# ALIZE-Speaker-Recognition/LIA_RAL

Measured on AMD Instinct MI355X. Metric: Gframe-Gaussian evals/s (UBM EM pass: LLK + full-posterior statistics), higher is better.
Workload: dtype f64; 1 GPU; TrainWorld EM: 2048-Gaussian diag UBM, 60-dim float32 frames, 10000000 frames per GPU resident in HBM, 1 EM iteration per step; gaussians=2048, dim=60, frames_per_gpu=10000000, partitioning=frames sharded per rank, one RCCL all-reduce of 247810 doubles per step

## Files before the change

lia_ral_amd/csrc/devutil.h:

```cpp
#pragma once
#include <hip/hip_runtime.h>
#include <stdint.h>

typedef double d4 __attribute__((ext_vector_type(4)));

#define MFMA_F64(a, b, c) __builtin_amdgcn_mfma_f64_16x16x4f64((a), (b), (c), 0, 0, 0)

#define GMMIV_NEG_BIG (-1.0e300)
#define GMMIV_ZERO_LLK (-745.1332191019412)
#define GMMIV_PAD_LOGIT (-1.0e9)

__device__ __forceinline__ double gexp(double x)
{
    x = fmax(x, -750.0);
    const double n = __builtin_rint(x * 1.4426950408889634074);
    double r = __builtin_fma(n, -6.93147180369123816490e-01, x);
    r = __builtin_fma(n, -1.90821492927058770002e-10, r);
    double p = 1.6059043836821613e-10;
    p = __builtin_fma(p, r, 2.08767569878681e-09);
    p = __builtin_fma(p, r, 2.505210838544172e-08);
    p = __builtin_fma(p, r, 2.755731922398589e-07);
    p = __builtin_fma(p, r, 2.7557319223985893e-06);
    p = __builtin_fma(p, r, 2.48015873015873e-05);
    p = __builtin_fma(p, r, 1.984126984126984e-04);
// ... 15 lines not shown
{
    x = fmax(x, -750.0);
    const double k = __builtin_rint(x * 46.16624130844683);
    double r = __builtin_fma(k, -0.021660849219188094, x);
    r = __builtin_fma(k, -1.733101967801894e-10, r);
    const int ki = (int)k;
    const double tj = tab[ki & 31];
    double p = 1.984126984126984e-04;
    p = __builtin_fma(p, r, 1.388888888888889e-03);
    p = __builtin_fma(p, r, 8.333333333333333e-03);
    p = __builtin_fma(p, r, 4.1666666666666664e-02);
    p = __builtin_fma(p, r, 1.6666666666666666e-01);
    p = __builtin_fma(p, r, 0.5);
    p = __builtin_fma(p, r, 1.0);
    p = p * r;
    return __builtin_ldexp(__builtin_fma(tj, p, tj), ki >> 5);
}

__device__ __forceinline__ double gexp_scaled(double x, int E, const double *tab)
{
    x = fmax(x, -4.0e7);
    const double k = __builtin_rint(x * 46.16624130844683);
    double r = __builtin_fma(k, -0.021660849219188094, x);
    r = __builtin_fma(k, -1.733101967801894e-10, r);
    const int ki = (int)k;
    const double tj = tab[ki & 31];
    double p = 1.984126984126984e-04;
    p = __builtin_fma(p, r, 1.388888888888889e-03);
    p = __builtin_fma(p, r, 8.333333333333333e-03);
    p = __builtin_fma(p, r, 4.1666666666666664e-02);
    p = __builtin_fma(p, r, 1.6666666666666666e-01);
    p = __builtin_fma(p, r, 0.5);
    p = __builtin_fma(p, r, 1.0);
    p = p * r;
    int n = (ki >> 5) - E;
    n = n < -2000 ? -2000 : n;
    return __builtin_ldexp(__builtin_fma(tj, p, tj), n);
}
#ifndef GEXP_TAB_BITS
#define GEXP_TAB_BITS 11
#endif
#define GEXP_TAB_N (1 << GEXP_TAB_BITS)
#if GEXP_TAB_BITS == 11
#define GEXP_TAB_SCALE 2954.639443740597
#define GEXP_TAB_HI 0.00033845076904981397
#define GEXP_TAB_LO 2.7079718246904592e-12
#define GEXP_TAB_LN2N 0.00033845077175778578
#elif GEXP_TAB_BITS == 6
#define GEXP_TAB_SCALE 92.33248261689366
#define GEXP_TAB_HI 0.010830424609594047
#define GEXP_TAB_LO 8.66550983900947e-11
#define GEXP_TAB_LN2N 0.010830424696249145
#else
#error "GEXP_TAB_BITS must be 6 or 11"
#endif
__device__ __forceinline__ void gexp_tab_init(double *tab, int tid, int nthreads)
{
    for (int j = tid; j < GEXP_TAB_N; j += nthreads) tab[j] = exp2((double)j * (1.0 / GEXP_TAB_N));
}
__device__ __forceinline__ double gexp_tab_poly(double r)
{
#if GEXP_TAB_BITS == 11
    double p = 1.6666666666666666e-01;
#else
    double p = 8.333333333333333e-03;
    p = __builtin_fma(p, r, 4.1666666666666664e-02);
    p = __builtin_fma(p, r, 1.6666666666666666e-01);
#endif
    p = __builtin_fma(p, r, 0.5);
    p = __builtin_fma(p, r, 1.0);
    return p * r;
}
__device__ __forceinline__ void gexp_tab_reduce(double x, int &ki, double &r)
{
    const double k = __builtin_rint(x * GEXP_TAB_SCALE);
#ifdef GEXP_TAB_TWO_STEP
    r = __builtin_fma(k, -GEXP_TAB_HI, x);
    r = __builtin_fma(k, -GEXP_TAB_LO, r);
#else
    r = __builtin_fma(k, -GEXP_TAB_LN2N, x);
#endif
    ki = (int)k;
}
__device__ __forceinline__ double gexp_tab_finish(int ki, double r, int E, const double *tab)
{
    const double tj = tab[ki & (GEXP_TAB_N - 1)];
    return __builtin_ldexp(__builtin_fma(tj, gexp_tab_poly(r), tj), (ki >> GEXP_TAB_BITS) - E);
}
__device__ __forceinline__ double gexp_tab_scaled(double x, int E, const double *tab)
{
    int ki;
    double r;
    gexp_tab_reduce(x, ki, r);
    return gexp_tab_finish(ki, r, E, tab);
}
__device__ __forceinline__ int gexp_tab_exponent(double x)
{
    return ((int)__builtin_rint(x * GEXP_TAB_SCALE)) >> GEXP_TAB_BITS;
}
__device__ __forceinline__ int gexp_exponent(double x)
{
    x = fmax(x, -4.0e7);
    return ((int)__builtin_rint(x * 46.16624130844683)) >> 5;
}

template <int CTRL> __device__ __forceinline__ int dpp_i32(int v) { return __builtin_amdgcn_update_dpp(0, v, CTRL, 0xf, 0xf, false); }
__device__ __forceinline__ int row_max_i32(int v)
{
    int o;
    o = dpp_i32<0x128>(v); v = o > v ? o : v;
    o = dpp_i32<0x124>(v); v = o > v ? o : v;
    o = dpp_i32<0x122>(v); v = o > v ? o : v;
    o = dpp_i32<0x121>(v); v = o > v ? o : v;
    return v;
}

__device__ __forceinline__ int row_min_i32(int v)
{
    int o;
    o = dpp_i32<0x128>(v); v = o < v ? o : v;
    o = dpp_i32<0x124>(v); v = o < v ? o : v;
    o = dpp_i32<0x122>(v); v = o < v ? o : v;
    o = dpp_i32<0x121>(v); v = o < v ? o : v;
    return v;
}

__device__ __forceinline__ void wave_argmax_f64(double &v, int &c)
{
#define GMMIV_ARGMAX_STEP(CTRL)                                                                    \
    {                                                                                              \
        const int ohi = dpp_i32<CTRL>(__double2hiint(v)), olo = dpp_i32<CTRL>(__double2loint(v)); \
        const int oc = dpp_i32<CTRL>(c);                                                           \
        const double ov = __hiloint2double(ohi, olo);                                              \
        if (ov > v || (ov == v && oc < c)) { v = ov; c = oc; }                                     \
    }
    GMMIV_ARGMAX_STEP(0x128)
    GMMIV_ARGMAX_STEP(0x124)
    GMMIV_ARGMAX_STEP(0x122)
    GMMIV_ARGMAX_STEP(0x121)
#undef GMMIV_ARGMAX_STEP
    const double v0 = __hiloint2double(__builtin_amdgcn_readlane(__double2hiint(v), 0), __builtin_amdgcn_readlane(__double2loint(v), 0));
    const int c0 = __builtin_amdgcn_readlane(c, 0);
    double wv = v0;
    int wc = c0;
#pragma unroll
    for (int r = 1; r < 4; ++r) {
        const double ov = __hiloint2double(__builtin_amdgcn_readlane(__double2hiint(v), 16 * r), __builtin_amdgcn_readlane(__double2loint(v), 16 * r));
        const int oc = __builtin_amdgcn_readlane(c, 16 * r);
        if (ov > wv || (ov == wv && oc < wc)) { wv = ov; wc = oc; }
    }
    v = wv;
    c = wc;
}

__device__ __forceinline__ double dpp_f64_0x128(double v) { return __hiloint2double(dpp_i32<0x128>(__double2hiint(v)), dpp_i32<0x128>(__double2loint(v))); }
__device__ __forceinline__ double dpp_f64_0x124(double v) { return __hiloint2double(dpp_i32<0x124>(__double2hiint(v)), dpp_i32<0x124>(__double2loint(v))); }
__device__ __forceinline__ double dpp_f64_0x122(double v) { return __hiloint2double(dpp_i32<0x122>(__double2hiint(v)), dpp_i32<0x122>(__double2loint(v))); }
__device__ __forceinline__ double dpp_f64_0x121(double v) { return __hiloint2double(dpp_i32<0x121>(__double2hiint(v)), dpp_i32<0x121>(__double2loint(v))); }
__device__ __forceinline__ double readlane_f64u(double v, int l)
{
    return __hiloint2double(__builtin_amdgcn_readlane(__double2hiint(v), l), __builtin_amdgcn_readlane(__double2loint(v), l));
}
__device__ __forceinline__ double wave_sum_f64_dpp(double v)
{
    v += dpp_f64_0x128(v); v += dpp_f64_0x124(v); v += dpp_f64_0x122(v); v += dpp_f64_0x121(v);
    return (readlane_f64u(v, 0) + readlane_f64u(v, 16)) + (readlane_f64u(v, 32) + readlane_f64u(v, 48));
}
__device__ __forceinline__ double half_sum_f64_dpp(double v, bool hi)
{
    v += dpp_f64_0x128(v); v += dpp_f64_0x124(v); v += dpp_f64_0x122(v); v += dpp_f64_0x121(v);
// ... 75 lines not shown
```

lia_ral_amd/csrc/gmm_kernels.hip:

```cpp
#include <atomic>
#include "devutil.h"
#include "lds_attr.h"
#include "gmm_kernels.h"

typedef double d2v __attribute__((ext_vector_type(2)));

__device__ __forceinline__ void gmm_const_one(int c, int C, int D, const double *__restrict__ w, const double *__restrict__ mean,
                                              const double *__restrict__ iv, double *__restrict__ a, double *__restrict__ logwcst)
{
    if (c >= C) { a[c] = GMMIV_NEG_BIG; logwcst[c] = GMMIV_NEG_BIG; return; }
    double sl = 0.0, sm = 0.0;
    for (int d = 0; d < D; ++d) {
        double v = iv[(size_t)c * D + d], m = mean[(size_t)c * D + d];
        sl += log(v);
        sm += m * m * v;
    }
    double lw = (w[c] > 0.0) ? log(w[c]) : GMMIV_NEG_BIG;
    double lc = lw - 0.5 * D * 1.8378770664093454836 + 0.5 * sl;
    lc = fmax(lc, GMMIV_NEG_BIG);
    logwcst[c] = lc;
    a[c] = fmax(lc - 0.5 * sm, GMMIV_NEG_BIG);
}
__global__ void k_gmm_const(int C, int Cp, int D, const double *__restrict__ w,
                            const double *__restrict__ mean, const double *__restrict__ iv,
                            double *__restrict__ a, double *__restrict__ logwcst)
{
    int c = blockIdx.x * blockDim.x + threadIdx.x;
    if (c >= Cp) return;
    gmm_const_one(c, C, D, w, mean, iv, a, logwcst);
}
__global__ void k_gmm_const_batch(int C, int Cp, int D, const double *__restrict__ w, long sw, const double *__restrict__ mean, long sm,
                                  const double *__restrict__ iv, long si, double *__restrict__ a, double *__restrict__ logwcst)
{
    const int c = blockIdx.x * blockDim.x + threadIdx.x;
    const size_t g = blockIdx.y;
    if (c >= Cp) return;
    gmm_const_one(c, C, D, w + g * sw, mean + g * sm, iv + g * si, a + g * Cp, logwcst + g * Cp);
}

__device__ __forceinline__ double gmm_pack_one(long e, int C, int D, int KS, const double *__restrict__ mean,
                                               const double *__restrict__ iv, const double *__restrict__ a)
{
    const int NR = 2 * KS + 2;
    int lane = e & 63;
    int row = (e >> 6) % NR;
    int ct = (e >> 6) / NR;
    int j = lane & 15, q = lane >> 4;
    int c = ct * 16 + j;
    double v = 0.0;
    if (row < 2 * KS) {
        int s = row < KS ? row : row - KS;
        int k = 4 * s + q;
        if (c < C && k < D) {
            double ivv = iv[(size_t)c * D + k];
            v = row < KS ? mean[(size_t)c * D + k] * ivv : -0.5 * ivv;
        }
    } else if (row == 2 * KS) {
        v = c < C ? fmax(a[c], GMMIV_PAD_LOGIT) : GMMIV_PAD_LOGIT;
    } else {
        v = q == 0 ? (c < C ? fmax(a[c], GMMIV_PAD_LOGIT) : GMMIV_PAD_LOGIT) : (q == 1 ? -1.0 : 0.0);
    }
    return v;
}
__global__ void k_gmm_pack(int C, int D, int KS, int nct, const double *__restrict__ mean,
                           const double *__restrict__ iv, const double *__restrict__ a,
                           double *__restrict__ Pt)
{
    long e = (long)blockIdx.x * blockDim.x + threadIdx.x;
    long total = (long)nct * (2 * KS + 2) * 64;
    if (e >= total) return;
    Pt[e] = gmm_pack_one(e, C, D, KS, mean, iv, a);
}
__global__ void k_gmm_pack_batch(int C, int Cp, int D, int KS, int nct, const int *__restrict__ ids, const double *__restrict__ mean, long sm,
                                 const double *__restrict__ iv, long si, const double *__restrict__ a, double *__restrict__ Pt)
{
    long e = (long)blockIdx.x * blockDim.x + threadIdx.x;
    long total = (long)nct * (2 * KS + 2) * 64;
    if (e >= total) return;
    const size_t g = (size_t)ids[blockIdx.y];
    Pt[(size_t)blockIdx.y * total + e] = gmm_pack_one(e, C, D, KS, mean + g * sm, iv + g * si, a + g * Cp);
}

__global__ void k_gmm_transpose(int C, int Cp, int D, const double *__restrict__ mean,
                                const double *__restrict__ iv, double *__restrict__ meanT,
                                double *__restrict__ ivT)
{
    long e = (long)blockIdx.x * blockDim.x + threadIdx.x;
    if (e >= (long)D * Cp) return;
    int c = e % Cp, d = e / Cp;
    meanT[e] = c < C ? mean[(size_t)c * D + d] : 0.0;
    ivT[e] = c < C ? iv[(size_t)c * D + d] : 0.0;
}

#define TOPC_CAP 256
#define GMMIV_MIN_FRAME_EXP (-1076)
#ifndef K1_ABL
#define K1_ABL 0
#endif
#ifndef K1_PLAIN_SHARED
#define K1_PLAIN_SHARED 1
#endif
template <int KS, typename XT, int NW, int MODE, bool MM = false>
__global__ __launch_bounds__(NW * 64, 2) void k_llk_mfma(const void *__restrict__ x, long T, long ldx, int D,
                                                  const double *__restrict__ Pt, int nct,
                                                  double *__restrict__ lse_out, int use_glds, int dbg,
                                                  double *__restrict__ zbuf, long nfb, int *__restrict__ eit,
                                                  double *__restrict__ inv_out, int *__restrict__ efin_out,
                                                  const gmmiv_model_tile *__restrict__ tiles, long pt_stride)
{
    constexpr bool WZ = MODE == 1, TC = MODE == 2;
    static_assert(!MM || (MODE != 2 && NW == 8), "a model per segment: plain and stored-likelihood modes, 8 waves");
    constexpr int NR = 2 * KS + 2;
    constexpr int GT = 2;
    constexpr int TILE_D = GT * NR * 64;
    constexpr int PIECES = TILE_D * 8 / 1024;
    extern __shared__ __attribute__((aligned(16))) char smem[];
    double *buf0 = (double *)smem;
    double *buf1 = buf0 + TILE_D;
    double *etab = buf1 + TILE_D;
    int *ccnt = (int *)(etab + GEXP_TAB_N);

    const int tid = threadIdx.x, lane = tid & 63, wave = tid >> 6;
    const int i16 = lane & 15, q = lane >> 4;
    long tb0 = (long)blockIdx.x * (NW * 32);
    long wlo = 0, whi = 0, olo = 0, ohi = 0;
    if constexpr (MM) {
        const gmmiv_model_tile me = tiles[blockIdx.x];
        tb0 = me.first; wlo = me.lo; whi = me.hi; olo = me.lo - me.pad_lo; ohi = me.hi + me.pad_hi;
        Pt += (size_t)me.model * pt_stride;
    }
    const long tb = tb0 + wave * 32;
    gexp_tab_init(etab, tid, NW * 64);
    if (TC) ccnt[tid >> 1] = 0;

    constexpr int NA = TC ? KS : 2 * KS;
    double A[2][NA];
#pragma unroll
    for (int h = 0; h < 2; ++h) {
        const long t = tb + h * 16 + i16;
#pragma unroll
        for (int s = 0; s < KS; ++s) {
            const int k = 4 * s + q;
            double v = 0.0;
            if ((MM ? (t >= wlo && t < whi) : t < T) && k < D) v = feat_load<XT>::get(x, t * ldx + k);
            A[h][s] = v;
            if (!TC) A[h][NA - KS + s] = v * v;
        }
    }

    const int ntiles = nct / GT;
    auto stage = [&](double *dst, int tile) {
        const char *src = (const char *)(Pt + (size_t)tile * TILE_D);
        if (use_glds) {
            if (PIECES % NW == 0) {
#pragma unroll
                for (int j = 0; j < PIECES / NW; ++j) {
                    const int p = wave + NW * j;
                    __builtin_amdgcn_global_load_lds(
                        (const __attribute__((address_space(1))) void *)(src + p * 1024 + lane * 16),
                        (__attribute__((address_space(3))) void *)((char *)dst + p * 1024), 16, 0, 0);
                }
            } else {
                for (int p = wave; p < PIECES; p += NW)
                    __builtin_amdgcn_global_load_lds(
                        (const __attribute__((address_space(1))) void *)(src + p * 1024 + lane * 16),
                        (__attribute__((address_space(3))) void *)((char *)dst + p * 1024), 16, 0, 0);
            }
        } else {
            for (int p = wave; p < PIECES; p += NW) {
                uint4 v = *(const uint4 *)(src + p * 1024 + lane * 16);
                *(uint4 *)((char *)dst + p * 1024 + lane * 16) = v;
            }
        }
    };

    double sacc[2][4];
    int E[2][4], nref[2][4];
#pragma unroll
    for (int h = 0; h < 2; ++h)
#pragma unroll
        for (int r = 0; r < 4; ++r) { sacc[h][r] = 0.0; E[h][r] = -(1 << 30); nref[h][r] = -(1 << 30); }

    const bool late = NW == 8 && ((wave >> 1) & 1);
    float thf[2][4], lmaxf[2][4];
#pragma unroll
    for (int h = 0; h < 2; ++h)
#pragma unroll
        for (int r = 0; r < 4; ++r) { thf[h][r] = -__builtin_inff(); lmaxf[h][r] = -__builtin_inff(); }
    d4 acc[GT][2];
    auto mfma_phase = [&](const double *cur) __attribute__((always_inline)) {
    double zv = 0.0;
    if (TC) asm volatile("" : "+v"(zv));
#pragma unroll
    for (int g = 0; g < GT; ++g) {
        const double a = cur[(g * NR + 2 * KS) * 64 + lane];
        acc[g][0] = (d4){a, a, a, a};
        acc[g][1] = acc[g][0];
    }
#pragma unroll
    for (int s = 0; s < 2 * KS; ++s) {
        const double b0 = cur[(0 * NR + s) * 64 + lane];
        const double b1 = cur[(1 * NR + s) * 64 + lane];
        double a0, a1;
        if (TC && s >= KS && !(K1_ABL & 256)) { a0 = __builtin_fma(A[0][s - KS], A[0][s - KS], zv); a1 = __builtin_fma(A[1][s - KS], A[1][s - KS], zv); }
        else if (TC && s >= KS) { a0 = A[0][s - KS]; a1 = A[1][s - KS]; }
        else { a0 = A[0][s < NA ? s : 0]; a1 = A[1][s < NA ? s : 0]; }
        acc[0][0] = MFMA_F64(a0, b0, acc[0][0]);
        acc[1][0] = MFMA_F64(a0, b1, acc[1][0]);
        acc[0][1] = MFMA_F64(a1, b0, acc[0][1]);
        acc[1][1] = MFMA_F64(a1, b1, acc[1][1]);
    }
    };
    auto epi_phase = [&](int te) __attribute__((always_inline)) {
        if (K1_ABL & 1) {
#pragma unroll
            for (int g = 0; g < GT; ++g)
#pragma unroll
                for (int h = 0; h < 2; ++h) asm volatile("" ::"v"(acc[g][h]));
            return;
        }
        if (TC) {
#ifndef TC_SCHED
#define TC_SCHED 1
#endif
            const bool refresh = TC_SCHED == 0 ? (te < 8 || (te < 16 && (te & 1) == 1) || (te < 32 && (te & 3) == 3) || (te & 7) == 7 || te == ntiles - 1)
                                               : ((te & (te + 1)) == 0 || te == ntiles - 1);
            const int kth = dbg > 0 ? dbg : 16;
#pragma unroll
            for (int h = 0; h < 2; ++h) {
                int nm[4], k0[4], k1[4];
                bool hit0[4], hit1[4];
                bool grow = false;
                if (!(K1_ABL & 128))
#pragma unroll
                for (int r = 0; r < 4; ++r)
                    lmaxf[h][r] = fmaxf(lmaxf[h][r], (float)fmax(acc[0][h][r], acc[1][h][r]));
                if (refresh && !(K1_ABL & 128)) {
#pragma unroll
                    for (int r = 0; r < 4; ++r) {
                        const int fb = __float_as_int(lmaxf[h][r]);
                        int key = ((fb ^ ((fb >> 31) & 0x7fffffff)) & ~15) | i16;
                        if (kth <= 8) {
                            for (int i = 1; i < kth; ++i) {
                                const int mx = row_max_i32(key);
                                key = key == mx ? (int)0x80000000 : key;
                            }
                            key = row_max_i32(key);
                        } else {
                            for (int i = kth; i < 16; ++i) {
                                const int mn = row_min_i32(key);
                                key = key == mn ? 0x7fffffff : key;
                            }
                            key = row_min_i32(key);
                        }
                        const float f = __int_as_float(key ^ ((key >> 31) & 0x7fffffff));
                        thf[h][r] = __builtin_fmaf(-__builtin_fabsf(f), 0x1p-17f, f);
                    }
                }
                int slot[4];
#pragma unroll
                for (int r = 0; r < 4; ++r) {
                    const double thd = (double)thf[h][r];
                    hit0[r] = !(K1_ABL & 64) && acc[0][h][r] >= thd;
                    hit1[r] = !(K1_ABL & 64) && acc[1][h][r] >= thd;
                    slot[r] = 0;
                    if (hit0[r] || hit1[r])
                        slot[r] = __hip_atomic_fetch_add(ccnt + (wave * 32 + q) + (h * 16 + 4 * r), (hit0[r] ? 1 : 0) + (hit1[r] ? 1 : 0), __ATOMIC_RELAXED,
                                                         __HIP_MEMORY_SCOPE_WORKGROUP);
                }
#pragma unroll
                for (int r = 0; r < 4; ++r) {
                    if (hit0[r] || hit1[r]) {
                        double *rp = zbuf + 2 * ((size_t)(tb + q + h * 16 + 4 * r) * TOPC_CAP + slot[r]);
                        if (hit0[r] && slot[r] < TOPC_CAP) {
                            d2v rec; rec[0] = acc[0][h][r]; rec[1] = __longlong_as_double((long long)(32 * te + i16));
                            *(d2v *)rp = rec;
                        }
                        const int s1 = slot[r] + (hit0[r] ? 1 : 0);
                        if (hit1[r] && s1 < TOPC_CAP) {
                            d2v rec; rec[0] = acc[1][h][r]; rec[1] = __longlong_as_double((long long)(32 * te + 16 + i16));
                            *(d2v *)(rp + (hit0[r] ? 2 : 0)) = rec;
                        }
                    }
                }
                __builtin_amdgcn_sched_barrier(0);
#pragma unroll
                for (int r = 0; r < 4; ++r) {
                    double r0, r1;
                    gexp_tab_reduce(acc[0][h][r], k0[r], r0);
                    gexp_tab_reduce(acc[1][h][r], k1[r], r1);
                    acc[0][h][r] = r0;
                    acc[1][h][r] = r1;
                    const int km = k0[r] > k1[r] ? k0[r] : k1[r];
                    nm[r] = km >> GEXP_TAB_BITS;
                    grow |= nm[r] - E[h][r] >= 64;
                }
                if (__builtin_amdgcn_ballot_w64(grow) != 0) {
#pragma unroll
                    for (int r = 0; r < 4; ++r) {
                        nm[r] = row_max_i32(nm[r]);
                        if (nm[r] - E[h][r] >= 64) {
                            int sh = E[h][r] - nm[r];
                            sh = sh < -2000 ? -2000 : sh;
                            sacc[h][r] = __builtin_ldexp(sacc[h][r], sh);
                            E[h][r] = nm[r];
                        }
                    }
                }
#pragma unroll
                for (int r = 0; r < 4; ++r) {
                    const double e0 = gexp_tab_finish(k0[r], acc[0][h][r], E[h][r], etab);
                    const double e1 = gexp_tab_finish(k1[r], acc[1][h][r], E[h][r], etab);
                    sacc[h][r] += (hit0[r] ? 0.0 : e0) + (hit1[r] ? 0.0 : e1);
                }
            }
            return;
        }
        if (WZ || (MODE == 0 && K1_PLAIN_SHARED)) {
            int nm[2][4], k0[2][4], k1[2][4];
            bool grow = false;
#pragma unroll
            for (int h = 0; h < 2; ++h)
#pragma unroll
                for (int r = 0; r < 4; ++r) {
                    double r0, r1;
                    gexp_tab_reduce(acc[0][h][r], k0[h][r], r0);
                    gexp_tab_reduce(acc[1][h][r], k1[h][r], r1);
                    acc[0][h][r] = r0;
                    acc[1][h][r] = r1;
                    const int km = k0[h][r] > k1[h][r] ? k0[h][r] : k1[h][r];
                    nm[h][r] = km >> GEXP_TAB_BITS;
                    grow |= nm[h][r] - E[h][r] >= 64;
                }
            if (__builtin_amdgcn_ballot_w64(grow) != 0) {
#pragma unroll
                for (int h = 0; h < 2; ++h)
#pragma unroll
                    for (int r = 0; r < 4; ++r) {
                        if (!(K1_ABL & 8)) nm[h][r] = row_max_i32(nm[h][r]);
                        if (nm[h][r] - E[h][r] >= 64) {
                            int sh = E[h][r] - nm[h][r];
                            sh = sh < -2000 ? -2000 : sh;
                            sacc[h][r] = __builtin_ldexp(sacc[h][r], sh);
                            E[h][r] = nm[h][r];
                        }
                    }
            }
#pragma unroll
            for (int h = 0; h < 2; ++h)
#pragma unroll
                for (int r = 0; r < 4; ++r) {
                    const double e0 = gexp_tab_finish(k0[h][r], acc[0][h][r], E[h][r], (K1_ABL & 2) ? etab - (k0[h][r] & (GEXP_TAB_N - 1)) : etab);
                    const double e1 = gexp_tab_finish(k1[h][r], acc[1][h][r], E[h][r], (K1_ABL & 2) ? etab - (k1[h][r] & (GEXP_TAB_N - 1)) : etab);
                    sacc[h][r] += e0 + e1;
                    acc[0][h][r] = e0;
                    acc[1][h][r] = e1;
                }
            if (!WZ) return;
            if (!late) asm volatile("s_waitcnt vmcnt(0)" ::: "memory");
            double *zw = zbuf + ((((size_t)(te * GT)) * nfb + (tb >> 4)) * 64 + lane) * 4;
            if (K1_ABL & 4) {
#pragma unroll
                for (int g = 0; g < GT; ++g)
#pragma unroll
                    for (int h = 0; h < 2; ++h) asm volatile("" ::"v"(acc[g][h]));
                return;
            }
            if constexpr (MM) {
                typedef int i4 __attribute__((ext_vector_type(4)));
                int *ew = eit + (size_t)te * (nfb * 16) + tb + 4 * q;
#pragma unroll
                for (int h = 0; h < 2; ++h) {
                    const long b0 = tb + 16 * h;
                    if (b0 >= olo && b0 + 16 <= ohi) {
#pragma unroll
                        for (int g = 0; g < GT; ++g) __builtin_nontemporal_store(acc[g][h], (d4 *)(zw + ((size_t)g * nfb + h) * 256));
                        if (i16 == 0) *(i4 *)(ew + h * 16) = (i4){E[h][0], E[h][1], E[h][2], E[h][3]};
                    } else if (b0 + 16 > olo && b0 < ohi) {
#pragma unroll
                        for (int r = 0; r < 4; ++r) {
                            const long t = b0 + q + 4 * r;
                            if (t >= olo && t < ohi) {
#pragma unroll
                                for (int g = 0; g < GT; ++g) zw[((size_t)g * nfb + h) * 256 + r] = acc[g][h][r];
                                if (i16 == 0) ew[h * 16 + r] = E[h][r];
                            }
                        }
                    }
                }
                return;
            }
#pragma unroll
            for (int g = 0; g < GT; ++g)
#pragma unroll
                for (int h = 0; h < 2; ++h) __builtin_nontemporal_store(acc[g][h], (d4 *)(zw + ((size_t)g * nfb + h) * 256));
            if (i16 == 0 && !(K1_ABL & 32)) {
                typedef int i4 __attribute__((ext_vector_type(4)));
                int *ew = eit + (size_t)te * (nfb * 16) + tb + 4 * q;
#pragma unroll
                for (int h = 0; h < 2; ++h) *(i4 *)(ew + h * 16) = (i4){E[h][0], E[h][1], E[h][2], E[h][3]};
            }
            return;
        }
        int nm[2][4];
        bool grow = false;
#pragma unroll
        for (int h = 0; h < 2; ++h)
#pragma unroll
            for (int r = 0; r < 4; ++r) {
                nm[h][r] = gexp_tab_exponent(fmax(acc[0][h][r], acc[1][h][r]));
                grow |= nm[h][r] - E[h][r] >= 64;
            }
        if (__builtin_amdgcn_ballot_w64(grow) != 0) {
#pragma unroll
            for (int h = 0; h < 2; ++h)
#pragma unroll
                for (int r = 0; r < 4; ++r)
                    if (nm[h][r] - E[h][r] >= 64) {
                        int sh = E[h][r] - nm[h][r];
                        sh = sh < -2000 ? -2000 : sh;
                        sacc[h][r] = __builtin_ldexp(sacc[h][r], sh);
                        E[h][r] = nm[h][r];
                    }
        }
        unsigned need = 0;
#pragma unroll
        for (int h = 0; h < 2; ++h)
#pragma unroll
            for (int r = 0; r < 4; ++r) {
                nref[h][r] = nm[h][r] > nref[h][r] ? nm[h][r] : nref[h][r];
                need |= (__builtin_amdgcn_ballot_w64(nm[h][r] > nref[h][r] - 57) != 0 ? 1u : 0u) << (h * 4 + r);
            }
        if (__builtin_popcount(need) > 3) {
#pragma unroll
            for (int h = 0; h < 2; ++h)
#pragma unroll
                for (int r = 0; r < 4; ++r)
                    sacc[h][r] += gexp_tab_scaled(acc[0][h][r], E[h][r], etab) + gexp_tab_scaled(acc[1][h][r], E[h][r], etab);
        } else if (need) {
#pragma unroll
            for (int h = 0; h < 2; ++h)
#pragma unroll
                for (int r = 0; r < 4; ++r)
                    if (need & (1u << (h * 4 + r)))
                        sacc[h][r] += gexp_tab_scaled(acc[0][h][r], E[h][r], etab) + gexp_tab_scaled(acc[1][h][r], E[h][r], etab);
        }
    };
    stage(buf0, 0);
    __syncthreads();
    auto step = [&](int tl, bool staged, bool is_late, bool first) __attribute__((always_inline)) {
        double *cur = (tl & 1) ? buf1 : buf0;
        double *nxt = (tl & 1) ? buf0 : buf1;
        if (staged && (TC || dbg < 2) && !(K1_ABL & 16)) stage(nxt, tl + 1);
        if (!is_late) {
            mfma_phase(cur);
            epi_phase(tl);
        } else {
            if (!first) epi_phase(tl - 1);
            mfma_phase(cur);
        }
        if (WZ) {
            if (is_late) asm volatile("s_waitcnt vmcnt(0)" ::: "memory");
            if (!(K1_ABL & 16)) asm volatile("s_waitcnt lgkmcnt(0)\n\ts_barrier" ::: "memory");
        } else {
            __syncthreads();
        }
    };
    if (!late) {
        for (int tl = 0; tl + 1 < ntiles; ++tl) step(tl, true, false, false);
        if (ntiles > 0) step(ntiles - 1, false, false, false);
    } else {
        if (ntiles > 1) step(0, true, true, true);
        for (int tl = 1; tl + 1 < ntiles; ++tl) step(tl, true, true, false);
        if (ntiles > 0) step(ntiles - 1, false, true, ntiles == 1);
    }
    if (late && ntiles > 0) epi_phase(ntiles - 1);
#pragma unroll
    for (int h = 0; h < 2; ++h)
#pragma unroll
        for (int r = 0; r < 4; ++r) {
            int Em = E[h][r];
#pragma unroll
            for (int o = 1; o < 16; o <<= 1) { const int oe = __shfl_xor(Em, o, 64); Em = oe > Em ? oe : Em; }
            int sh = E[h][r] - Em;
            sh = sh < -2000 ? -2000 : sh;
            double sv = __builtin_ldexp(sacc[h][r], sh);
#pragma unroll
            for (int o = 1; o < 16; o <<= 1) sv += shfl_xor_f64(sv, o);
            const long t = tb + h * 16 + q + 4 * r;
            if (TC) {
                if (i16 == 0 && t < T) { lse_out[t] = (double)thf[h][r]; inv_out[t] = sv; efin_out[t] = Em; }
                continue;
            }
            if (i16 == 0 && (MM ? (t >= wlo && t < whi) : t < T)) {
                const bool ok = sv > 0.0 && sv < __builtin_inf() && Em > GMMIV_MIN_FRAME_EXP;
                lse_out[t] = ok ? log(sv) + (double)Em * 0.693147180559945309417 : -__builtin_inf();
                if (WZ) { inv_out[t] = ok ? 1.0 / sv : 0.0; efin_out[t] = ok ? Em : 0; }
            }
        }
    if (TC) {
        __syncthreads();
        const long t = (long)blockIdx.x * (NW * 32) + tid;
        if (tid < NW * 32 && t < T) eit[t] = ccnt[tid];
    }
}

__global__ __launch_bounds__(256) void k_llk_finalize(const double *__restrict__ lse, long T, double lo,
                                                     double hi, double *__restrict__ llk_out,
                                                     double *__restrict__ partial)
{
    __shared__ double red[3][4];
    double sc = 0.0, sr = 0.0, sn = 0.0;
    for (long t = (long)blockIdx.x * blockDim.x + threadIdx.x; t < T; t += (long)gridDim.x * blockDim.x) {
        const double v = lse[t];
        const double c = fmin(fmax(v, lo), hi);
        if (llk_out) llk_out[t] = c;
        sc += c;
        const bool fin = v > -__builtin_inf() && v < __builtin_inf();
        sr += fin ? v : 0.0;
        sn += fin ? 1.0 : 0.0;
    }
    sc = wave_sum_f64(sc);
    sr = wave_sum_f64(sr);
    sn = wave_sum_f64(sn);
    const int lane = threadIdx.x & 63, wave = threadIdx.x >> 6;
    if (lane == 0) { red[0][wave] = sc; red[1][wave] = sr; red[2][wave] = sn; }
    __syncthreads();
    if (threadIdx.x == 0) {
        partial[3 * blockIdx.x] = red[0][0] + red[0][1] + red[0][2] + red[0][3];
        partial[3 * blockIdx.x + 1] = red[1][0] + red[1][1] + red[1][2] + red[1][3];
        partial[3 * blockIdx.x + 2] = red[2][0] + red[2][1] + red[2][2] + red[2][3];
    }
}

__global__ __launch_bounds__(256) void k_count_dead(const double *__restrict__ lse, long T, unsigned long long *__restrict__ cnt)
{
    unsigned n = 0;
    for (long t = (long)blockIdx.x * blockDim.x + threadIdx.x; t < T; t += (long)gridDim.x * blockDim.x) {
        const double v = lse[t];
        n += (v > -__builtin_inf() && v < __builtin_inf()) ? 0u : 1u;
    }
    const unsigned long long b = __ballot(n > 0);
    if (b == 0) return;
    for (int o = 32; o > 0; o >>= 1) n += __shfl_xor(n, o, 64);
    if ((threadIdx.x & 63) == 0) atomicAdd(cnt, (unsigned long long)n);
}
// ... 538 lines not shown
    if (!(l > -__builtin_inf())) l = __builtin_inf();
    for (int c = threadIdx.x; c < C; c += 256) {
        double acc = 0.0;
        for (int d = 0; d < D; ++d) {
            const double dx = xs[d] - meanT[(size_t)d * Cp + c];
            acc = __builtin_fma(dx * dx, ivT[(size_t)d * Cp + c], acc);
        }
        const double z = __builtin_fma(-0.5, acc, lwc[c]);
        gamma[t * C + c] = z == z ? exp(z - l) : 0.0;
    }
}

template <typename XT>
__global__ __launch_bounds__(256) void k_frame_moments(const void *__restrict__ x, long T, long ldx, int D,
                                                       double *__restrict__ partial)
{
    __shared__ double red[2][4][64];
    const int d = threadIdx.x & 63, rs = threadIdx.x >> 6;
    double s = 0.0, ss = 0.0;
    for (int d0 = 0; d0 < D; d0 += 64) {
        s = 0.0; ss = 0.0;
        const int dd = d0 + d;
        if (dd < D)
            for (long t = (long)blockIdx.x * 4 + rs; t < T; t += (long)gridDim.x * 4) {
                const double v = feat_load<XT>::raw(x, t * ldx + dd);
                s += v;
                ss = __builtin_fma(v, v, ss);
            }
        red[0][rs][d] = s;
        red[1][rs][d] = ss;
        __syncthreads();
        if (rs == 0 && dd < D) {
            partial[(size_t)blockIdx.x * 2 * D + dd] = red[0][0][d] + red[0][1][d] + red[0][2][d] + red[0][3][d];
            partial[(size_t)blockIdx.x * 2 * D + D + dd] = red[1][0][d] + red[1][1][d] + red[1][2][d] + red[1][3][d];
        }
        __syncthreads();
    }
}
__global__ __launch_bounds__(256) void k_moments_reduce(const double *__restrict__ partial, int nb, int n, double *__restrict__ acc)
{
    __shared__ double red[4][64];
    const int lane = threadIdx.x & 63, slot = threadIdx.x >> 6;
    const int e = blockIdx.x * 4 + slot;
    double s = 0.0;
    if (e < n)
        for (int b = lane; b < nb; b += 64) s += partial[(size_t)b * n + e];
    red[slot][lane] = s;
    __syncthreads();
    if (lane == 0 && e < n) {
        double t = 0.0;
        for (int l = 0; l < 64; ++l) t += red[slot][l];
        acc[e] += t;
    }
}

#define HIPCHK(e)                                                         \
    do {                                                                  \
        hipError_t _e = (e);                                              \
        if (_e != hipSuccess) return (int)_e;                             \
    } while (0)

int gmmk_ks_for_dim(int D)
{
    if (D <= 16) return 4;
    if (D <= 32) return 8;
    if (D <= 60) return 15;
    if (D <= 80) return 20;
    return D <= GMMK_MAX_DIM ? GMMK_KS_GENERIC : 0;
}
int gmmk_rl_for_ks(int KS) { return ((4 * KS + 2 + 31) / 32) * 32; }

int gmmk_pack_model(hipStream_t st, int C, int D, int KS, int nct, int Cp64, const double *w, const double *mean,
                    const double *iv, double *a, double *lwc, double *Pt, double *meanT, double *ivT)
{
    const int Cp = Cp64 > nct * 16 ? Cp64 : nct * 16;
    k_gmm_const<<<(Cp + 255) / 256, 256, 0, st>>>(C, Cp, D, w, mean, iv, a, lwc);
    long total = (long)nct * (2 * KS + 2) * 64;
    if (KS != GMMK_KS_GENERIC) k_gmm_pack<<<(unsigned)((total + 255) / 256), 256, 0, st>>>(C, D, KS, nct, mean, iv, a, Pt);
    long tt = (long)D * Cp64;
    k_gmm_transpose<<<(unsigned)((tt + 255) / 256), 256, 0, st>>>(C, Cp64, D, mean, iv, meanT, ivT);
    return (int)hipGetLastError();
}

template <int KS, typename XT, int NW, int MODE>
static int launch_llk(hipStream_t st, const void *x, long T, long ldx, int D, const double *Pt, int nct,
                      double *lse, int use_glds, const gmmk_zview &z = gmmk_zview{})
{
    constexpr int NR = 2 * KS + 2;
    const size_t lds = 2 * 2 * NR * 64 * sizeof(double) + GEXP_TAB_N * sizeof(double) + (MODE == 2 ? NW * 32 * sizeof(int) : 0);
    HIPCHK((gmmiv_lds_attr<k_llk_mfma<KS, XT, NW, MODE>>(lds)));
    const unsigned grid = (unsigned)((T + NW * 32 - 1) / (NW * 32));
    k_llk_mfma<KS, XT, NW, MODE><<<grid, NW * 64, lds, st>>>(x, T, ldx, D, Pt, nct, lse, use_glds & 1, use_glds >> 8, z.zbuf, z.nfb, z.eit, z.inv, z.efin, nullptr, 0);
    return (int)hipGetLastError();
}

template <int KS, typename XT, int MODE>
static int launch_llk_models(hipStream_t st, const void *x, long ldx, int D, const double *Pt, long pt_stride, int nct, const gmmiv_model_tile *tiles,
                             long ntiles, double *lse, int use_glds, const gmmk_zview &z)
{
    constexpr int NR = 2 * KS + 2;
    const size_t lds = 2 * 2 * NR * 64 * sizeof(double) + GEXP_TAB_N * sizeof(double);
    HIPCHK((gmmiv_lds_attr<k_llk_mfma<KS, XT, 8, MODE, true>>(lds)));
    k_llk_mfma<KS, XT, 8, MODE, true><<<(unsigned)ntiles, 8 * 64, lds, st>>>(x, 0, ldx, D, Pt, nct, lse, use_glds & 1, 0, z.zbuf, z.nfb, z.eit, z.inv, z.efin, tiles, pt_stride);
    return (int)hipGetLastError();
}
#define MM_CASE(K, MODE)                                                                                                  \
    case K:                                                                                                               \
        return x_f64 ? launch_llk_models<K, double, MODE>(st, x, ldx, D, Pt, pt_stride, nct, tiles, ntiles, lse, use_glds, z) \
                     : launch_llk_models<K, float, MODE>(st, x, ldx, D, Pt, pt_stride, nct, tiles, ntiles, lse, use_glds, z);
int gmmk_llk_models(hipStream_t st, int KS, int x_f64, const void *x, long ldx, int D, const double *Pt, long pt_stride, int nct,
                    const gmmiv_model_tile *tiles, long ntiles, double *lse, int use_glds)
{
    if (ntiles <= 0) return 0;
    const gmmk_zview z = {};
    switch (KS) {
        MM_CASE(4, 0) MM_CASE(8, 0) MM_CASE(15, 0)
    }
    return -1;
}
int gmmk_llk_z_models(hipStream_t st, int KS, int x_f64, const void *x, long ldx, int D, const double *Pt, long pt_stride, int nct,
                      const gmmiv_model_tile *tiles, long ntiles, double *lse, int use_glds, const gmmk_zview &z)
{
    if (ntiles <= 0) return 0;
    switch (KS) {
        MM_CASE(4, 1) MM_CASE(8, 1) MM_CASE(15, 1)
    }
    return -1;
}
#undef MM_CASE

int gmmk_const_models(hipStream_t st, int G, int C, int Cp, int D, const double *w, long sw, const double *mean, long sm, const double *iv,
                      long si, double *a, double *lwc)
{
    if (G <= 0) return 0;
    k_gmm_const_batch<<<dim3((unsigned)((Cp + 255) / 256), (unsigned)G), 256, 0, st>>>(C, Cp, D, w, sw, mean, sm, iv, si, a, lwc);
    return (int)hipGetLastError();
}
int gmmk_pack_models(hipStream_t st, int n, const int *ids, int C, int Cp, int D, int KS, int nct, const double *mean, long sm,
                     const double *iv, long si, const double *a, double *Pt)
{
    if (n <= 0) return 0;
    const long total = (long)nct * (2 * KS + 2) * 64;
    k_gmm_pack_batch<<<dim3((unsigned)((total + 255) / 256), (unsigned)n), 256, 0, st>>>(C, Cp, D, KS, nct, ids, mean, sm, iv, si, a, Pt);
    return (int)hipGetLastError();
}

__global__ __launch_bounds__(256) void k_llk_seg_finalize(const double *__restrict__ lse, const long *__restrict__ sb, double lo, double hi,
                                                         double *__restrict__ llk_out, double *__restrict__ seg_sum,
                                                         double *__restrict__ seg_llk)
{
    __shared__ double red[3][4];
    const int s = blockIdx.x;
    const long b = sb[s], e = sb[s + 1];
    double sc = 0.0, sr = 0.0, sn = 0.0;
    for (long t = b + threadIdx.x; t < e; t += 256) {
        const double v = lse[t];
        const double c = fmin(fmax(v, lo), hi);
        if (llk_out) llk_out[t] = c;
        sc += c;
        const bool fin = v > -__builtin_inf() && v < __builtin_inf();
        sr += fin ? v : 0.0;
        sn += fin ? 1.0 : 0.0;
    }
    sc = wave_sum_f64(sc);
    sr = wave_sum_f64(sr);
    sn = wave_sum_f64(sn);
    const int lane = threadIdx.x & 63, wave = threadIdx.x >> 6;
    if (lane == 0) { red[0][wave] = sc; red[1][wave] = sr; red[2][wave] = sn; }
    __syncthreads();
    if (threadIdx.x == 0) {
        if (seg_sum) seg_sum[s] = red[0][0] + red[0][1] + red[0][2] + red[0][3];
        if (seg_llk) {
            seg_llk[2 * s] = red[1][0] + red[1][1] + red[1][2] + red[1][3];
            seg_llk[2 * s + 1] = red[2][0] + red[2][1] + red[2][2] + red[2][3];
        }
    }
}
int gmmk_llk_seg_finalize(hipStream_t st, const double *lse, const long *sb, long nseg, double lo, double hi, double *llk_out, double *seg_sum,
                          double *seg_llk)
{
    if (nseg <= 0) return 0;
    k_llk_seg_finalize<<<(unsigned)nseg, 256, 0, st>>>(lse, sb, lo, hi, llk_out, seg_sum, seg_llk);
    return (int)hipGetLastError();
}

__device__ __forceinline__ double map_ml_weight(double n, double count) { return count > 0.0 ? n / count : 0.0; }
__device__ __forceinline__ double map_mean_one(double ml, double m0, double w, double w0c, double cnt, int method, int mean_adapt, double mean_reg,
// ... 716 lines not shown
```

Measured before the change: 128.5 Gframe-Gaussian/s.

## Use buffer-load-to-LDS staging, split exp table gather, and add MFMA schedule hints

Makes the staging path a template parameter and replaces global_load_lds with raw buffer loads to LDS through a buffer resource descriptor, using scalar tile offsets. Splits the exp table lookup into a separate gather pass ahead of the polynomial evaluation and adds sched_group_barrier hints that interleave LDS reads with MFMA and VALU work. Also swaps the inline asm waitcnt for builtins, with the barrier waiting only on LDS counters. The goal is to cut address arithmetic and hide LDS and table latency behind compute, at the cost of more register pressure and a fragile scheduling dependence; the MM models path with per-model Pt stride may not be covered by the descriptor size.

```diff
diff --git a/lia_ral_amd/csrc/devutil.h b/lia_ral_amd/csrc/devutil.h
--- a/lia_ral_amd/csrc/devutil.h
+++ b/lia_ral_amd/csrc/devutil.h
@@ -121,10 +121,14 @@
 #endif
     ki = (int)k;
 }
+__device__ __forceinline__ double gexp_tab_gather(int ki, const double *tab) { return tab[ki & (GEXP_TAB_N - 1)]; }
+__device__ __forceinline__ double gexp_tab_apply(double tj, int ki, double r, int E)
+{
+    return __builtin_ldexp(__builtin_fma(tj, gexp_tab_poly(r), tj), (ki >> GEXP_TAB_BITS) - E);
+}
 __device__ __forceinline__ double gexp_tab_finish(int ki, double r, int E, const double *tab)
 {
-    const double tj = tab[ki & (GEXP_TAB_N - 1)];
-    return __builtin_ldexp(__builtin_fma(tj, gexp_tab_poly(r), tj), (ki >> GEXP_TAB_BITS) - E);
+    return gexp_tab_apply(gexp_tab_gather(ki, tab), ki, r, E);
 }
 __device__ __forceinline__ double gexp_tab_scaled(double x, int E, const double *tab)
 {
diff --git a/lia_ral_amd/csrc/gmm_kernels.hip b/lia_ral_amd/csrc/gmm_kernels.hip
--- a/lia_ral_amd/csrc/gmm_kernels.hip
+++ b/lia_ral_amd/csrc/gmm_kernels.hip
@@ -100,10 +100,16 @@
 #ifndef K1_PLAIN_SHARED
 #define K1_PLAIN_SHARED 1
 #endif
-template <int KS, typename XT, int NW, int MODE, bool MM = false>
+__device__ __forceinline__ void k1_wait_vm0() { __builtin_amdgcn_s_waitcnt(0x0F70); }
+__device__ __forceinline__ void k1_barrier_lds_only()
+{
+    __builtin_amdgcn_s_waitcnt(0xC07F);
+    __builtin_amdgcn_s_barrier();
+}
+template <int KS, typename XT, int NW, int MODE, bool MM = false, bool GLDS = true>
 __global__ __launch_bounds__(NW * 64, 2) void k_llk_mfma(const void *__restrict__ x, long T, long ldx, int D,
                                                   const double *__restrict__ Pt, int nct,
-                                                  double *__restrict__ lse_out, int use_glds, int dbg,
+                                                  double *__restrict__ lse_out, int dbg,
                                                   double *__restrict__ zbuf, long nfb, int *__restrict__ eit,
                                                   double *__restrict__ inv_out, int *__restrict__ efin_out,
                                                   const gmmiv_model_tile *__restrict__ tiles, long pt_stride)
@@ -149,22 +155,23 @@
     }
 
     const int ntiles = nct / GT;
+    [[maybe_unused]] const __amdgpu_buffer_rsrc_t ptr_rsrc =
+        __builtin_amdgcn_make_buffer_rsrc((void *)Pt, 0, (int)((unsigned)nct * (unsigned)(NR * 64 * 8)), 0x00020000);
     auto stage = [&](double *dst, int tile) {
         const char *src = (const char *)(Pt + (size_t)tile * TILE_D);
-        if (use_glds) {
+        if constexpr (GLDS) {
+            const int soff = tile * (TILE_D * 8);
             if (PIECES % NW == 0) {
 #pragma unroll
                 for (int j = 0; j < PIECES / NW; ++j) {
                     const int p = wave + NW * j;
-                    __builtin_amdgcn_global_load_lds(
-                        (const __attribute__((address_space(1))) void *)(src + p * 1024 + lane * 16),
-                        (__attribute__((address_space(3))) void *)((char *)dst + p * 1024), 16, 0, 0);
+                    __builtin_amdgcn_raw_ptr_buffer_load_lds(ptr_rsrc, (__attribute__((address_space(3))) void *)((char *)dst + p * 1024), 16,
+                                                         wave * 1024 + lane * 16, soff + NW * j * 1024, 0, 0);
                 }
             } else {
                 for (int p = wave; p < PIECES; p += NW)
-                    __builtin_amdgcn_global_load_lds(
-                        (const __attribute__((address_space(1))) void *)(src + p * 1024 + lane * 16),
-                        (__attribute__((address_space(3))) void *)((char *)dst + p * 1024), 16, 0, 0);
+                    __builtin_amdgcn_raw_ptr_buffer_load_lds(ptr_rsrc, (__attribute__((address_space(3))) void *)((char *)dst + p * 1024), 16,
+                                                         p * 1024 + lane * 16, soff, 0, 0);
             }
         } else {
             for (int p = wave; p < PIECES; p += NW) {
@@ -209,6 +216,14 @@
         acc[1][0] = MFMA_F64(a0, b1, acc[1][0]);
         acc[0][1] = MFMA_F64(a1, b0, acc[0][1]);
         acc[1][1] = MFMA_F64(a1, b1, acc[1][1]);
+    }
+    if (!TC) {
+        __builtin_amdgcn_sched_group_barrier(0x100, 5, 1);
+#pragma unroll
+        for (int s = 0; s < 2 * KS; ++s) {
+            __builtin_amdgcn_sched_group_barrier(0x008, 4, 1);
+            __builtin_amdgcn_sched_group_barrier(0x100, 1, 1);
+        }
     }
     };
     auto epi_phase = [&](int te) __attribute__((always_inline)) {
@@ -346,18 +361,32 @@
                         }
                     }
             }
+            double tj0[2][4], tj1[2][4];
 #pragma unroll
             for (int h = 0; h < 2; ++h)
 #pragma unroll
                 for (int r = 0; r < 4; ++r) {
-                    const double e0 = gexp_tab_finish(k0[h][r], acc[0][h][r], E[h][r], (K1_ABL & 2) ? etab - (k0[h][r] & (GEXP_TAB_N - 1)) : etab);
-                    const double e1 = gexp_tab_finish(k1[h][r], acc[1][h][r], E[h][r], (K1_ABL & 2) ? etab - (k1[h][r] & (GEXP_TAB_N - 1)) : etab);
+                    tj0[h][r] = gexp_tab_gather(k0[h][r], (K1_ABL & 2) ? etab - (k0[h][r] & (GEXP_TAB_N - 1)) : etab);
+                    tj1[h][r] = gexp_tab_gather(k1[h][r], (K1_ABL & 2) ? etab - (k1[h][r] & (GEXP_TAB_N - 1)) : etab);
+                }
+#pragma unroll
+            for (int i = 0; i < 16; ++i) {
+                __builtin_amdgcn_sched_group_barrier(0x002, 2, 0);
+                __builtin_amdgcn_sched_group_barrier(0x100, 1, 0);
+            }
+            __builtin_amdgcn_sched_group_barrier(0x002, 400, 0);
+#pragma unroll
+            for (int h = 0; h < 2; ++h)
+#pragma unroll
+                for (int r = 0; r < 4; ++r) {
+                    const double e0 = gexp_tab_apply(tj0[h][r], k0[h][r], acc[0][h][r], E[h][r]);
+                    const double e1 = gexp_tab_apply(tj1[h][r], k1[h][r], acc[1][h][r], E[h][r]);
                     sacc[h][r] += e0 + e1;
                     acc[0][h][r] = e0;
                     acc[1][h][r] = e1;
                 }
             if (!WZ) return;
-            if (!late) asm volatile("s_waitcnt vmcnt(0)" ::: "memory");
+            if (!late) k1_wait_vm0();
             double *zw = zbuf + ((((size_t)(te * GT)) * nfb + (tb >> 4)) * 64 + lane) * 4;
             if (K1_ABL & 4) {
 #pragma unroll
@@ -451,7 +480,7 @@
     auto step = [&](int tl, bool staged, bool is_late, bool first) __attribute__((always_inline)) {
         double *cur = (tl & 1) ? buf1 : buf0;
         double *nxt = (tl & 1) ? buf0 : buf1;
-        if (staged && (TC || dbg < 2) && !(K1_ABL & 16)) stage(nxt, tl + 1);
+        if (staged && !(K1_ABL & 16)) stage(nxt, tl + 1);
         if (!is_late) {
             mfma_phase(cur);
             epi_phase(tl);
@@ -460,8 +489,8 @@
             mfma_phase(cur);
         }
         if (WZ) {
-            if (is_late) asm volatile("s_waitcnt vmcnt(0)" ::: "memory");
-            if (!(K1_ABL & 16)) asm volatile("s_waitcnt lgkmcnt(0)\n\ts_barrier" ::: "memory");
+            if (is_late) k1_wait_vm0();
+            if (!(K1_ABL & 16)) k1_barrier_lds_only();
         } else {
             __syncthreads();
         }
@@ -1166,27 +1195,40 @@
     return (int)hipGetLastError();
 }
 
+template <int KS, typename XT, int NW, int MODE, bool GLDS>
+static int launch_llk_as(hipStream_t st, const void *x, long T, long ldx, int D, const double *Pt, int nct, double *lse, int dbg, const gmmk_zview &z)
+{
+    constexpr int NR = 2 * KS + 2;
+    const size_t lds = 2 * 2 * NR * 64 * sizeof(double) + GEXP_TAB_N * sizeof(double) + (MODE == 2 ? NW * 32 * sizeof(int) : 0);
+    HIPCHK((gmmiv_lds_attr<k_llk_mfma<KS, XT, NW, MODE, false, GLDS>>(lds)));
+    const unsigned grid = (unsigned)((T + NW * 32 - 1) / (NW * 32));
+    k_llk_mfma<KS, XT, NW, MODE, false, GLDS><<<grid, NW * 64, lds, st>>>(x, T, ldx, D, Pt, nct, lse, dbg, z.zbuf, z.nfb, z.eit, z.inv, z.efin, nullptr, 0);
+    return (int)hipGetLastError();
+}
 template <int KS, typename XT, int NW, int MODE>
 static int launch_llk(hipStream_t st, const void *x, long T, long ldx, int D, const double *Pt, int nct,
                       double *lse, int use_glds, const gmmk_zview &z = gmmk_zview{})
 {
+    return (use_glds & 1) ? launch_llk_as<KS, XT, NW, MODE, true>(st, x, T, ldx, D, Pt, nct, lse, use_glds >> 8, z)
+                          : launch_llk_as<KS, XT, NW, MODE, false>(st, x, T, ldx, D, Pt, nct, lse, use_glds >> 8, z);
+}
+
+template <int KS, typename XT, int MODE, bool GLDS>
+static int launch_llk_models_as(hipStream_t st, const void *x, long ldx, int D, const double *Pt, long pt_stride, int nct, const gmmiv_model_tile *tiles,
+                                long ntiles, double *lse, const gmmk_zview &z)
+{
     constexpr int NR = 2 * KS + 2;
-    const size_t lds = 2 * 2 * NR * 64 * sizeof(double) + GEXP_TAB_N * sizeof(double) + (MODE == 2 ? NW * 32 * sizeof(int) : 0);
-    HIPCHK((gmmiv_lds_attr<k_llk_mfma<KS, XT, NW, MODE>>(lds)));
-    const unsigned grid = (unsigned)((T + NW * 32 - 1) / (NW * 32));
-    k_llk_mfma<KS, XT, NW, MODE><<<grid, NW * 64, lds, st>>>(x, T, ldx, D, Pt, nct, lse, use_glds & 1, use_glds >> 8, z.zbuf, z.nfb, z.eit, z.inv, z.efin, nullptr, 0);
-    return (int)hipGetLastError();
-}
-
+    const size_t lds = 2 * 2 * NR * 64 * sizeof(double) + GEXP_TAB_N * sizeof(double);
+    HIPCHK((gmmiv_lds_attr<k_llk_mfma<KS, XT, 8, MODE, true, GLDS>>(lds)));
+    k_llk_mfma<KS, XT, 8, MODE, true, GLDS><<<(unsigned)ntiles, 8 * 64, lds, st>>>(x, 0, ldx, D, Pt, nct, lse, 0, z.zbuf, z.nfb, z.eit, z.inv, z.efin, tiles, pt_stride);
+    return (int)hipGetLastError();
+}
 template <int KS, typename XT, int MODE>
 static int launch_llk_models(hipStream_t st, const void *x, long ldx, int D, const double *Pt, long pt_stride, int nct, const gmmiv_model_tile *tiles,
                              long ntiles, double *lse, int use_glds, const gmmk_zview &z)
 {
-    constexpr int NR = 2 * KS + 2;
-    const size_t lds = 2 * 2 * NR * 64 * sizeof(double) + GEXP_TAB_N * sizeof(double);
-    HIPCHK((gmmiv_lds_attr<k_llk_mfma<KS, XT, 8, MODE, true>>(lds)));
-    k_llk_mfma<KS, XT, 8, MODE, true><<<(unsigned)ntiles, 8 * 64, lds, st>>>(x, 0, ldx, D, Pt, nct, lse, use_glds & 1, 0, z.zbuf, z.nfb, z.eit, z.inv, z.efin, tiles, pt_stride);
-    return (int)hipGetLastError();
+    return (use_glds & 1) ? launch_llk_models_as<KS, XT, MODE, true>(st, x, ldx, D, Pt, pt_stride, nct, tiles, ntiles, lse, z)
+                          : launch_llk_models_as<KS, XT, MODE, false>(st, x, ldx, D, Pt, pt_stride, nct, tiles, ntiles, lse, z);
 }
 #define MM_CASE(K, MODE)                                                                                                  \
     case K:                                                                                                               \
```

Result: no change. 129.6 Gframe-Gaussian/s (median of 6 runs) (+0.9%).
